# bencebecsy/pta_replicator

Hardware: AMD Instinct MI355X
Metric: realizations/sec, 68 psr x 5000 TOAs GWB+RN+WN (higher is better)
Workload: dtype f64; 1 GPU; BASELINE.json config 3: the 68 pulsars of ng15_dict.json x 5000 synthetic TOAs - HD GWB (gw_log10_A of the dict) + per-pulsar power-law RN (dict values, 30 components) + per-backend EFAC / t2EQUAD / ECORR (dict values), on-chip Philox draws, 1024 realisations per step per GPU; n_toa_total=340000, Nf=3000, npts=600, parallelism=replica-shard x1

## Files before the change

include/pta_replicator_amd.h:

```cpp
#ifndef PTA_REPLICATOR_AMD_H
#define PTA_REPLICATOR_AMD_H

#include <stdint.h>

#ifdef __cplusplus
extern "C" {
#endif

#define PTA_ABI_VERSION 8

#define PTA_OK 0
#define PTA_E_ARG (-1)
#define PTA_E_HIP (-2)
#define PTA_E_NOTPD (-3)

int pta_abi_version(void);
const char *pta_last_error(void);
int pta_device_info(int *cu_count, int *wavefront, char *arch, int arch_len);



int pta_rng_philox_raw(const uint32_t *ctr, const uint32_t *key, int n, uint32_t *out, void *stream);

int pta_rng_fill_normal(uint64_t seed, uint64_t r0, int R, uint32_t stream_id, int npairs, int interleave,
// ... 49 lines not shown
int pta_potrf_batched_ex(double *A, int n, int64_t lda, int64_t strideA, int B, int32_t *info, int flags, void *stream);

int64_t pta_potrf_workspace_doubles(int n, int B, int flags);
int pta_potrf_batched_ws(double *A, int n, int64_t lda, int64_t strideA, int B, int32_t *info, int flags, double *work,
                         int64_t work_doubles, void *stream);

int pta_potrf_warmup(int nchain);

int64_t pta_potrf_ragged_plan_words(int B);
int pta_potrf_ragged_plan(const int32_t *n, const int64_t *off, const int64_t *ld, int B, int flags, int64_t *plan_host,
                          int64_t *work_doubles);
int pta_potrf_ragged(double *A, const int64_t *plan_host, const int64_t *plan_dev, int32_t *info, double *work,
                     int64_t work_doubles, void *stream);



int pta_gwb_twiddle(const double *sqrtC, int Nf, int npts, int i0, double inv_dt, double *T, int64_t ldt, void *stream);

int pta_gwb_idft(const double *w, int64_t ldw, int M, int Nf, const double *T, int64_t ldt, int npts, double *G0,
                 int64_t ldg, int algo, void *stream);

int64_t pta_gwb_twiddle_sym_size(int Nf, int npts, int variant, int64_t *rot_doubles);
int pta_gwb_twiddle_sym(const double *sqrtC, int Nf, int npts, int i0, double inv_dt, double *Tsym, double *rot,
                        int variant, void *stream);
int pta_gwb_idft_rng(uint64_t seed, uint64_t r0, int R, int P, int Nf, const double *Tsym, const double *rot, int npts,
                     double *G0, int64_t ldg, int variant, int rng_fast, void *stream);

int pta_gwb_czt_fits(int Nf, int npts, int i0);
int pta_gwb_czt_setup(const double *sqrtC, int Nf, int npts, int i0, double inv_dt, double *pre, double *FB, double *tw,
                      double *post, void *stream);
int pta_gwb_czt(uint64_t seed, uint64_t r0, const double *w, int64_t ldw, int R, int P, int Nf, int npts, int i0,
                const double *pre, const double *FB, const double *tw, const double *post, double *G0, int64_t ldg,
                int variant, int rng_fast, void *stream);

int pta_gwb_czt_scaled(uint64_t seed, uint64_t r0, const double *w, int64_t ldw, int R, int P, int Nf, int npts, int i0,
                       const double *pre, const double *FB, const double *tw, const double *post, double *G0, int64_t ldg,
                       int variant, int rng_fast, const double *scale, int64_t ld_scale, void *stream);
int pta_gwb_idft_rng_scaled(uint64_t seed, uint64_t r0, int R, int P, int Nf, const double *Tsym, const double *rot, int npts,
                            double *G0, int64_t ldg, int variant, int rng_fast, const double *scale, int64_t ld_scale, void *stream);
int pta_gwb_spectrum_scale(const double *f, const double *hcf0, int Nf, int R, const double *log10_A, const double *gamma, int turnover,
                           double f0, double beta, double power, double *scale, int64_t ld_scale, void *stream);
int pta_gwb_spectrum_scale_user(const int32_t *seg, const double *dx, const double *dxp, const double *hcf0, int Nf, int M, int R,
                                const double *log10_hc, int64_t ld_hc, double *scale, int64_t ld_scale, void *stream);

int pta_gwb_mix(const double *Mchol, int P, const double *G0, int R, int npts, int64_t ldg, double *G, int variant, void *stream);

int pta_gwb_orf_factor(const double *basis, int n_lm, int P, const double *clm, int64_t ld_clm, int R, double *Mchol, int32_t *info,
                       void *stream);
int pta_gwb_mix_batched(const double *Mchol, int64_t ld_m, int P, const double *G0, int R, int npts, int64_t ldg, double *G, int variant,
                        void *stream);

int pta_gwb_bracket(const double *ut, int npts, const double *toa_s, int N, int32_t *jlo, void *stream);

int pta_gwb_weights(const double *ut, int npts, const double *toa_s, const int32_t *jlo, int N, double *w, void *stream);

int pta_gwb_interp(const double *G, int64_t ldg, int P, int npts, const double *ut, const double *toa_s,
                   const int32_t *psr_of_toa, const int32_t *jlo, int N, int R, double scale, double *out,
                   int64_t ld_out, int accumulate, void *stream);

#define PTA_CGW_NPAR 18
int pta_cgw(const double *mjd, int N, const double *par_host, double *out, int accumulate, void *stream);

#define PTA_CW_NPAR 16
int pta_cw_catalog_workspace(int N, int ncw, int64_t *partial_doubles, int *nchunk);
int pta_cw_catalog(const double *mjd, int N, const double *par, int ncw, int psr_term, int mode, double tref,
                   double *partial_ws, double *out, int accumulate, void *stream);
// ... 298 lines not shown
```

pta_replicator_amd/_lib.py:

```python
import ctypes
import os
from ctypes import POINTER, c_char_p, c_double, c_int, c_int32, c_int64, c_uint32, c_uint64, c_void_p

import torch

_HERE = os.path.dirname(os.path.abspath(__file__))
LIB_PATH = os.environ.get("PTA_REPLICATOR_AMD_LIB") or os.path.join(_HERE, "libpta_replicator_amd.so")


class PtaError(RuntimeError):
    """A call into libpta_replicator_amd.so returned a PTA_E_* code."""


if not os.path.exists(LIB_PATH):
    raise ImportError(
        f"{LIB_PATH} is missing: build the HIP library first (python -m pta_replicator_amd.build, or "
        "__graft_entry__.build()). pta_replicator_amd has no CPU fallback.")

lib = ctypes.CDLL(LIB_PATH)

_P = c_void_p


class EnginePlan(ctypes.Structure):
# ... 71 lines not shown
    "pta_rng_fill_normal": (c_int, [c_uint64, c_uint64, c_int, c_uint32, c_int, c_int, _P, _P, c_int64, c_int, _P]),
    "pta_rng_fill_normal_blocks": (c_int, [c_uint64, c_uint64, c_int, c_uint32, c_int, _P, _P, c_int, _P, c_int64, c_int, _P]),
    "pta_rn_basis": (c_int, [_P, c_int, c_double, _P, _P, c_int, c_int, _P, c_int64, _P]),
    "pta_rn_synth": (c_int, [_P, c_int64, c_int, c_int, _P, c_int64, c_int, _P, c_int64, c_int, _P]),
    "pta_wn": (c_int, [_P, _P, _P, c_int, c_int, _P, _P, c_int64, c_int, _P, c_int64, c_int, _P]),
    "pta_quantize_epochs": (c_int, [_P, c_int, c_double, _P, _P, _P, POINTER(c_int)]),
    "pta_dot3_host": (c_int, [_P, c_int64, _P, _P]),
    "pta_pow_host": (c_int, [_P, c_double, c_int64, _P]),
    "pta_legacy_randn": (c_int, [_P, _P, _P, c_int, _P, _P, _P, _P, c_int]),
    "pta_ecorr": (c_int, [_P, _P, c_int, c_int, _P, c_int64, c_int, _P, c_int64, c_int, _P]),
    "pta_orf_pair_arguments": (c_int, [_P, c_int, _P, _P]),
    "pta_orf_hd": (c_int, [_P, c_int, _P, _P]),
    "pta_orf_basis": (c_int, [_P, _P, c_int, c_int, _P, _P]),
    "pta_orf_combine": (c_int, [_P, _P, c_int, c_int, _P, _P]),
    "pta_potrf_batched": (c_int, [_P, c_int, c_int, _P, _P]),
    "pta_potrf_batched_ex": (c_int, [_P, c_int, c_int64, c_int64, c_int, _P, c_int, _P]),
    "pta_potrf_workspace_doubles": (c_int64, [c_int, c_int, c_int]),
    "pta_potrf_batched_ws": (c_int, [_P, c_int, c_int64, c_int64, c_int, _P, c_int, _P, c_int64, _P]),
    "pta_potrf_warmup": (c_int, [c_int]),
    "pta_td_assemble_potrf": (c_int, [_P, _P, c_int, _P, _P, _P, _P, c_int, c_int64, c_int64, c_int, _P, c_int, _P, c_int64, _P]),
    "pta_potrf_ragged_plan_words": (c_int64, [c_int]),
    "pta_potrf_ragged_plan": (c_int, [_P, _P, _P, c_int, c_int, _P, POINTER(c_int64)]),
    "pta_potrf_ragged": (c_int, [_P, _P, _P, _P, _P, c_int64, _P]),
    "pta_gwb_twiddle": (c_int, [_P, c_int, c_int, c_int, c_double, _P, c_int64, _P]),
    "pta_gwb_idft": (c_int, [_P, c_int64, c_int, c_int, _P, c_int64, c_int, _P, c_int64, c_int, _P]),
    "pta_gwb_twiddle_sym_size": (c_int64, [c_int, c_int, c_int, POINTER(c_int64)]),
    "pta_gwb_twiddle_sym": (c_int, [_P, c_int, c_int, c_int, c_double, _P, _P, c_int, _P]),
    "pta_gwb_idft_rng": (c_int, [c_uint64, c_uint64, c_int, c_int, c_int, _P, _P, c_int, _P, c_int64, c_int, c_int, _P]),
    "pta_gwb_czt_fits": (c_int, [c_int, c_int, c_int]),
    "pta_gwb_czt_setup": (c_int, [_P, c_int, c_int, c_int, c_double, _P, _P, _P, _P, _P]),
    "pta_gwb_czt": (c_int, [c_uint64, c_uint64, _P, c_int64, c_int, c_int, c_int, c_int, c_int, _P, _P, _P, _P, _P, c_int64, c_int, c_int, _P]),
    "pta_gwb_czt_scaled": (c_int, [c_uint64, c_uint64, _P, c_int64, c_int, c_int, c_int, c_int, c_int, _P, _P, _P, _P, _P, c_int64, c_int, c_int,
                                   _P, c_int64, _P]),
    "pta_gwb_idft_rng_scaled": (c_int, [c_uint64, c_uint64, c_int, c_int, c_int, _P, _P, c_int, _P, c_int64, c_int, c_int, _P, c_int64, _P]),
    "pta_gwb_spectrum_scale": (c_int, [_P, _P, c_int, c_int, _P, _P, c_int, c_double, c_double, c_double, _P, c_int64, _P]),
    "pta_gwb_mix": (c_int, [_P, c_int, _P, c_int, c_int, c_int64, _P, c_int, _P]),
    "pta_gwb_orf_factor": (c_int, [_P, c_int, c_int, _P, c_int64, c_int, _P, _P, _P]),
    "pta_gwb_mix_batched": (c_int, [_P, c_int64, c_int, _P, c_int, c_int, c_int64, _P, c_int, _P]),
    "pta_gwb_bracket": (c_int, [_P, c_int, _P, c_int, _P, _P]),
    "pta_gwb_weights": (c_int, [_P, c_int, _P, _P, c_int, _P, _P]),
    "pta_gwb_interp": (c_int, [_P, c_int64, c_int, c_int, _P, _P, _P, _P, c_int, c_int, c_double, _P, c_int64, c_int, _P]),
    "pta_cgw": (c_int, [_P, c_int, _P, _P, c_int, _P]),
    "pta_cw_catalog_workspace": (c_int, [c_int, c_int, POINTER(c_int64), POINTER(c_int)]),
    "pta_cw_catalog": (c_int, [_P, c_int, _P, c_int, c_int, c_int, c_double, _P, _P, c_int, _P]),
    "pta_engine_rn_coef": (c_int, [c_uint64, c_uint64, c_int, c_int, c_int, _P, _P, c_int, _P]),
    "pta_engine_generate": (c_int, [POINTER(EnginePlan), POINTER(EngineTables), c_uint64, c_uint64, c_int, _P, c_int64, _P]),
    "pta_hyper_uniform": (c_int, [c_uint64, c_uint64, c_int, c_int, _P, _P, _P, _P]),
    "pta_engine_rn_coef_hyper": (c_int, [c_uint64, c_uint64, c_int, c_int, c_int, _P, _P, _P, _P, _P, _P, c_int, _P]),
    "pta_engine_generate_hyper": (c_int, [POINTER(EnginePlan), POINTER(EngineTables), POINTER(EngineHyper), c_uint64, c_uint64, c_int, _P,
                                          c_int64, _P]),
    "pta_cw_uniform": (c_int, [c_uint64, c_uint64, c_int, c_int, _P, _P, _P, _P]),
    "pta_engine_cw_params": (c_int, [POINTER(CwEngine), c_int, _P]),
    "pta_engine_cw_add": (c_int, [POINTER(EnginePlan), POINTER(CwEngine), c_int, _P, c_int64, c_int, _P]),
    "pta_cw_catalog_uniform": (c_int, [c_uint64, c_uint64, c_int, c_int, _P, _P, _P, _P]),
    "pta_engine_cw_catalog_params": (c_int, [POINTER(CwCatalogEngine), c_int, _P]),
    "pta_engine_cw_catalog_add": (c_int, [POINTER(EnginePlan), POINTER(CwCatalogEngine), c_int, _P, c_int64, c_int, _P]),
    "pta_bwm_uniform": (c_int, [c_uint64, c_uint64, c_int, _P, _P, _P, _P]),
    "pta_engine_bwm_params": (c_int, [POINTER(BwmEngine), c_int, _P]),
    "pta_engine_bwm_add": (c_int, [POINTER(EnginePlan), POINTER(BwmEngine), c_int, _P, c_int64, c_int, _P]),
    "pta_engine_wn_params": (c_int, [POINTER(WnHyper), c_int, _P]),
    "pta_engine_wn_add": (c_int, [POINTER(EnginePlan), POINTER(WnHyper), c_uint64, c_uint64, c_int, _P, c_int64, c_int, _P]),
    "pta_engine_synth": (c_int, [POINTER(EnginePlan), c_uint64, c_uint64, c_int, _P, c_int64, _P]),
    "pta_td_cov_assemble": (c_int, [_P, c_int64, c_int, c_int, _P, _P, _P, _P, _P, c_int64, _P]),
    "pta_td_cov_assemble_all": (c_int, [_P, c_int64, c_int, _P, _P, _P, _P, _P, _P, _P, _P, _P, c_int, c_int, _P]),
    "pta_td_cov_walk_items": (c_int64, [_P, c_int, c_int, c_int, _P]),
    "pta_td_cov_assemble_walk": (c_int, [_P, c_int64, c_int, _P, _P, _P, _P, _P, _P, _P, _P, _P, c_int, _P, c_int64, _P, c_int, _P]),
# ... 79 lines not shown
```

pta_replicator_amd/csrc/pta_czt_kernels.hip:

```cpp
#include "pta_common.h"
#include "pta_fft.h"

__global__ __launch_bounds__(PTA_FFT_THREADS) void k_czt_setup(const double *__restrict__ sqrtC, int Nf, int npts, int i0,
                                                               double inv_dt, double *__restrict__ pre,
                                                               double *__restrict__ FB, double *__restrict__ tw,
                                                               double *__restrict__ post) {
  __shared__ double re[PTA_FFT_PLANE], im[PTA_FFT_PLANE];
  const int tid = threadIdx.x;
  const int Kf = Nf - 2;
  const int64_t n = 2 * (int64_t)Nf - 2;
  for (int m = tid; m < PTA_FFT_N; m += PTA_FFT_THREADS) {
    double s, c;
    sincospi((double)(2 * m) / (double)PTA_FFT_N, &s, &c);
    tw[2 * m] = c;
    tw[2 * m + 1] = -s;
    double pr = 0.0, pi_ = 0.0;
    if (m < Kf) {
      int64_t k = m + 1, q = (k * k) % (2 * n);
      sincospi((double)q / (double)n, &s, &c);
      pr = sqrtC[k] * c;
      pi_ = sqrtC[k] * s;
    }
    pre[2 * m] = pr;
    pre[2 * m + 1] = pi_;
// ... 300 lines not shown
extern "C" int pta_gwb_czt_scaled(uint64_t seed, uint64_t r0, const double *w, int64_t ldw, int R, int P, int Nf, int npts, int i0,
                                  const double *pre, const double *FB, const double *tw, const double *post, double *G0, int64_t ldg,
                                  int variant, int rng_fast, const double *scale, int64_t ld_scale, void *stream) {
  PTA_REQUIRE(pre && FB && tw && post && G0 && scale, PTA_E_ARG, "pta_gwb_czt_scaled: NULL argument");
  PTA_REQUIRE(!w, PTA_E_ARG, "pta_gwb_czt_scaled: draws are generated on chip (w must be NULL)");
  (void)ldw;
  PTA_REQUIRE(R > 0 && P > 0 && P < (1 << 24) && npts > 0 && ldg >= npts, PTA_E_ARG, "pta_gwb_czt_scaled: R=%d P=%d npts=%d", R, P,
              npts);
  PTA_REQUIRE(czt_fits(Nf, npts, i0), PTA_E_ARG, "pta_gwb_czt_scaled: Nf=%d npts=%d i0=%d does not fit one 4096-point convolution", Nf,
              npts, i0);
  PTA_REQUIRE(ld_scale >= Nf - 1, PTA_E_ARG, "pta_gwb_czt_scaled: ld_scale=%lld < Nf - 1", (long long)ld_scale);
  int64_t M64 = (int64_t)R * P;
  PTA_REQUIRE(M64 < (1LL << 31), PTA_E_ARG, "pta_gwb_czt_scaled: R*P too large");
  const int M = (int)M64;
  PTA_REQUIRE(variant == 0 || variant == 1, PTA_E_ARG, "pta_gwb_czt_scaled: variant %d (0 or 1)", variant);
#define PTA_CZT_S(FASTV, FUSEV)                                                                                                     \
  hipLaunchKernelGGL((k_gwb_czt<true, FASTV, FUSEV, true>), dim3(M), dim3(PTA_FFT_THREADS), 0, pta_stream(stream), seed, r0, nullptr, \
                     0, M, P, Nf, npts, i0, pre, FB, tw, post, G0, ldg, scale, ld_scale, czt_last2(npts, i0))
  if (variant == 0) {
    if (rng_fast)
      PTA_CZT_S(true, PTA_CZT_FUSE_DEFAULT);
    else
      PTA_CZT_S(false, PTA_CZT_FUSE_DEFAULT);
  } else {
    if (rng_fast)
      PTA_CZT_S(true, 0);
    else
      PTA_CZT_S(false, 0);
  }
#undef PTA_CZT_S
  PTA_LAUNCH_CHECK();
  return PTA_OK;
}
```

pta_replicator_amd/csrc/pta_engine_kernels.hip:

```cpp
#include "pta_common.h"
#include "pta_rng.h"
#include "pta_mfma.h"

__global__ void k_engine_rn_coef(uint64_t seed, uint64_t r0, int R, int P, int K, const double *__restrict__ amp,
                                 double *__restrict__ coef, int fast) {
  pta_rng_stage_tables();
  __syncthreads();
  int idx = blockIdx.x * blockDim.x + threadIdx.x;
  int hp = K / 2;
  int total = R * P * hp;
  if (idx >= total) return;
  int p = idx % hp, ra = idx / hp;
  int a = ra % P, r = ra / P;
  double z0, z1;
  pta_normal_pair(seed, r0 + (uint64_t)r, pta_stream_id(PTA_STREAM_RN, (uint32_t)a), (uint32_t)p, z0, z1, fast);
  int64_t o = (int64_t)ra * K + 2 * p;
  coef[o] = amp[(int64_t)a * K + 2 * p] * z0;
  coef[o + 1] = amp[(int64_t)a * K + 2 * p + 1] * z1;
}

extern "C" int pta_engine_rn_coef(uint64_t seed, uint64_t r0, int R, int P, int K, const double *amp, double *coef, int rng_fast,
                                  void *stream) {
  PTA_REQUIRE(amp && coef, PTA_E_ARG, "pta_engine_rn_coef: NULL argument");
  PTA_REQUIRE(R > 0 && P > 0 && K > 0 && (K % 2) == 0, PTA_E_ARG, "pta_engine_rn_coef: R=%d P=%d K=%d (K must be even)", R, P, K);
// ... 361 lines not shown
  PTA_REQUIRE(!p.wn_a || p.wn_b, PTA_E_ARG, "pta_engine_synth: wn_b missing");
  PTA_REQUIRE(!p.wn_c || !p.wn_a, PTA_E_ARG, "pta_engine_synth: wn_c (single-deviate white noise) replaces wn_a / wn_b - pass one or the other");
  PTA_REQUIRE(!p.ecorr_toa || p.epoch_of, PTA_E_ARG, "pta_engine_synth: epoch_of missing");
  const int variant = p.synth_variant;
  const bool copies = variant == 16 || variant == 32 || variant == 48 || variant == 64;
  PTA_REQUIRE(variant == 0 || variant == 1 || variant == 2 || variant == 6 || copies || (variant >= 100 && variant <= 164), PTA_E_ARG,
              "pta_engine_synth: synth_variant %d does not exist (0, 1, 2, 6, 16, 32, 48, 64, 100 .. 164)", variant);
  if (variant != 6) {
    const int xcd = variant == 1 ? 0 : 1;
    const unsigned pad = variant >= 100 ? (unsigned)(variant - 100) * 1024u : 0u;
    const int64_t total = (int64_t)pta_cdiv(R, ENG_MR) * p.n_tiles, nwg = ((total + 7) >> 3) << 3;
    PTA_REQUIRE(nwg < (1LL << 31), PTA_E_ARG, "pta_engine_synth: %lld workgroups exceed one launch", (long long)nwg);
    const bool noidx = variant == 2 || (copies && ((variant - 16) & 16));
    const bool rnidx = !noidx && p.rn_k > 0 && p.ldf < (1LL << 28) && ((int64_t)p.rn_k * p.ldf + PTA_ENGINE_TILE) * 8 + 24 < (1LL << 32) &&
                       (int64_t)R * p.n_psr * p.rn_k * 8 < (1LL << 32);
    const bool generic = variant == 2 || (copies && ((variant - 16) & 32));
    const bool all = !generic && p.gw_npts > 0 && (p.wn_a || p.wn_c) && p.ecorr_toa;
    hipLaunchKernelGGL(synth_kernel(p.rng_fast != 0, p.wn_c != nullptr, rnidx, all), dim3((unsigned)nwg), dim3(PTA_ENGINE_TILE), pad,
                       pta_stream(stream), p, seed, r0, R, out, ld_out, xcd);
    PTA_LAUNCH_CHECK();
    return PTA_OK;
  }
  PTA_REQUIRE(!p.wn_c, PTA_E_ARG, "pta_engine_synth: the single-deviate white noise exists in the MFMA kernel only");
  PTA_REQUIRE(p.n_tiles <= 65535, PTA_E_ARG, "pta_engine_synth: %d tiles exceed the 2-D launch of the all-VALU kernel", p.n_tiles);
  hipLaunchKernelGGL(k_engine_synth<6>, dim3(pta_cdiv(R, ENG_RB), p.n_tiles), dim3(PTA_ENGINE_TILE), 0, pta_stream(stream), p, seed, r0, R,
                     out, ld_out, p.rng_fast ? 1 : 0);
  PTA_LAUNCH_CHECK();
  return PTA_OK;
}

extern "C" int pta_gwb_czt(uint64_t seed, uint64_t r0, const double *w, int64_t ldw, int R, int P, int Nf, int npts, int i0,
                           const double *pre, const double *FB, const double *tw, const double *post, double *G0, int64_t ldg,
                           int variant, int rng_fast, void *stream);
extern "C" int pta_gwb_idft_rng(uint64_t seed, uint64_t r0, int R, int P, int Nf, const double *Tsym, const double *rot, int npts,
                                double *G0, int64_t ldg, int variant, int rng_fast, void *stream);
extern "C" int pta_gwb_mix(const double *Mchol, int P, const double *G0, int R, int npts, int64_t ldg, double *G, int variant,
                           void *stream);
extern "C" int pta_gwb_mix_batched(const double *Mchol, int64_t ld_m, int P, const double *G0, int R, int npts, int64_t ldg, double *G,
                                   int variant, void *stream);

static int engine_generate(const char *fn, const pta_engine_plan *plan_host, const pta_engine_tables *tables_host,
                           const pta_engine_hyper *hyper, uint64_t seed, uint64_t r0, int R, double *out, int64_t ld_out, void *stream) {
  PTA_REQUIRE(plan_host && tables_host && out, PTA_E_ARG, "%s: NULL argument", fn);
  const pta_engine_hyper fixed{};
  const pta_engine_hyper &h = hyper ? *hyper : fixed;
  pta_engine_plan p = *plan_host;
  const pta_engine_tables &tb = *tables_host;
  int rc;
  if (p.rn_k > 0) {
    PTA_REQUIRE(tb.rn_amp && tb.ws_coef, PTA_E_ARG, "%s: red-noise amplitudes / workspace missing", fn);
    if (h.rn_log10_A) {
      PTA_REQUIRE(h.rn_gamma && h.rn_f && h.rn_tspan, PTA_E_ARG, "%s: rn_gamma / rn_f / rn_tspan missing", fn);
      rc = pta_engine_rn_coef_hyper(seed, r0, R, p.n_psr, p.rn_k, h.rn_f, h.rn_tspan, h.rn_log10_A, h.rn_gamma, tb.rn_amp, tb.ws_coef,
                                    p.rng_fast, stream);
    } else {
      rc = pta_engine_rn_coef(seed, r0, R, p.n_psr, p.rn_k, tb.rn_amp, tb.ws_coef, p.rng_fast, stream);
    }
    if (rc != PTA_OK) return rc;
    p.rn_coef = tb.ws_coef;
  }
  if (p.gw_npts > 0) {
    PTA_REQUIRE(tb.Mchol && tb.ws_G0 && tb.ws_G, PTA_E_ARG, "%s: GWB factor / workspace missing", fn);
    const double *scale = h.gw_scale;
    if (!scale && h.gw_log10_A) {
      PTA_REQUIRE(h.gw_gamma && h.gw_f && h.gw_hcf0 && h.ws_scale, PTA_E_ARG, "%s: gw_gamma / gw_f / gw_hcf0 / ws_scale missing", fn);
      rc = pta_gwb_spectrum_scale(h.gw_f, h.gw_hcf0, tb.gw_nf, R, h.gw_log10_A, h.gw_gamma, h.gw_turnover, h.gw_f0, h.gw_beta,
                                  h.gw_power, h.ws_scale, h.ld_gw_scale, stream);
      if (rc != PTA_OK) return rc;
      scale = h.ws_scale;
    }
    if (tb.use_czt) {
      PTA_REQUIRE(tb.czt_pre && tb.czt_FB && tb.czt_tw && tb.czt_post, PTA_E_ARG, "%s: chirp-z tables missing", fn);
      rc = scale ? pta_gwb_czt_scaled(seed, r0, nullptr, 0, R, p.n_psr, tb.gw_nf, p.gw_npts, tb.gw_i0, tb.czt_pre, tb.czt_FB, tb.czt_tw,
                                      tb.czt_post, tb.ws_G0, p.gw_npts, tb.czt_variant, p.rng_fast, scale, h.ld_gw_scale, stream)
                 : pta_gwb_czt(seed, r0, nullptr, 0, R, p.n_psr, tb.gw_nf, p.gw_npts, tb.gw_i0, tb.czt_pre, tb.czt_FB, tb.czt_tw,
                               tb.czt_post, tb.ws_G0, p.gw_npts, tb.czt_variant, p.rng_fast, stream);
    } else {
      PTA_REQUIRE(tb.Tsym && tb.rot, PTA_E_ARG, "%s: DFT-GEMM tables missing", fn);
      rc = scale ? pta_gwb_idft_rng_scaled(seed, r0, R, p.n_psr, tb.gw_nf, tb.Tsym, tb.rot, p.gw_npts, tb.ws_G0, p.gw_npts, tb.idft_variant,
                                           p.rng_fast, scale, h.ld_gw_scale, stream)
                 : pta_gwb_idft_rng(seed, r0, R, p.n_psr, tb.gw_nf, tb.Tsym, tb.rot, p.gw_npts, tb.ws_G0, p.gw_npts, tb.idft_variant,
                                    p.rng_fast, stream);
    }
    if (rc != PTA_OK) return rc;
    rc = h.gw_mchol ? pta_gwb_mix_batched(h.gw_mchol, h.ld_gw_mchol, p.n_psr, tb.ws_G0, R, p.gw_npts, p.gw_npts, tb.ws_G, tb.mix_variant, stream)
                    : pta_gwb_mix(tb.Mchol, p.n_psr, tb.ws_G0, R, p.gw_npts, p.gw_npts, tb.ws_G, tb.mix_variant, stream);
    if (rc != PTA_OK) return rc;
    p.gw_G = tb.ws_G;
  }
  return pta_engine_synth(&p, seed, r0, R, out, ld_out, stream);
}

extern "C" int pta_engine_generate(const pta_engine_plan *plan_host, const pta_engine_tables *tables_host, uint64_t seed, uint64_t r0,
                                   int R, double *out, int64_t ld_out, void *stream) {
  return engine_generate("pta_engine_generate", plan_host, tables_host, nullptr, seed, r0, R, out, ld_out, stream);
}

extern "C" int pta_engine_generate_hyper(const pta_engine_plan *plan_host, const pta_engine_tables *tables_host,
                                         const pta_engine_hyper *hyper_host, uint64_t seed, uint64_t r0, int R, double *out,
                                         int64_t ld_out, void *stream) {
  PTA_REQUIRE(hyper_host, PTA_E_ARG, "pta_engine_generate_hyper: NULL argument");
  return engine_generate("pta_engine_generate_hyper", plan_host, tables_host, hyper_host, seed, r0, R, out, ld_out, stream);
}
```

pta_replicator_amd/csrc/pta_fft.h:

```cpp
#pragma once
#include "pta_rng.h"

#define PTA_FFT_N 4096
#define PTA_FFT_THREADS 512
#define PTA_FFT_PHYS(i) ((i) + ((i) >> 3) + (((i) >> 9) << 3))
#define PTA_FFT_PLANE (PTA_FFT_N + PTA_FFT_N / 8 + 64)

struct pta_cplx {
  double re, im;
};

PTA_HD pta_cplx pta_cmul(pta_cplx a, pta_cplx b) { return {fma(a.re, b.re, -(a.im * b.im)), fma(a.re, b.im, a.im * b.re)}; }
PTA_HD pta_cplx pta_cadd(pta_cplx a, pta_cplx b) { return {a.re + b.re, a.im + b.im}; }
PTA_HD pta_cplx pta_csub(pta_cplx a, pta_cplx b) { return {a.re - b.re, a.im - b.im}; }
template <bool INV>
PTA_HD pta_cplx pta_cmuli(pta_cplx a) {
  return INV ? pta_cplx{-a.im, a.re} : pta_cplx{a.im, -a.re};
}

template <bool INV>
PTA_HD void pta_dft8(pta_cplx *v) {
  const double h = 0.70710678118654752440;
  pta_cplx a0 = pta_cadd(v[0], v[4]), a4 = pta_csub(v[0], v[4]);
  pta_cplx a1 = pta_cadd(v[1], v[5]), a5 = pta_csub(v[1], v[5]);
// ... 115 lines not shown
  pta_cplx d0 = pta_cadd(a4, t6), d1 = pta_cadd(t5, t7);
  v[1] = pta_cadd(d0, d1);
}

template <int LOG2S>
PTA_HD void pta_fft_core_inv_out01(pta_cplx *v, const pta_cplx *w) {
  if (LOG2S > 0) {
#pragma unroll
    for (int q = 1; q < 8; ++q) v[q] = pta_cmul(v[q], pta_cplx{w[q].re, -w[q].im});
  }
  pta_dft8_inv_out01(v);
}

template <bool INV, int LOG2S>
PTA_HD void pta_fft_pass_w(double *re, double *im, int tid, const pta_cplx *w) {
  int b, o;
  pta_fft_map<LOG2S>(tid, b, o);
  pta_cplx v[8];
  pta_fft_load<LOG2S>(re, im, b, o, v);
  pta_fft_core<INV, LOG2S>(v, w);
  pta_fft_store<LOG2S>(re, im, b, o, v);
}

template <bool INV, int LOG2S, int TW = 3>
PTA_HD void pta_fft_pass(double *re, double *im, const double *tw, int tid) {
  int b, o;
  pta_fft_map<LOG2S>(tid, b, o);
  pta_cplx v[8], w[8];
  pta_fft_twiddles<LOG2S, TW>(tw, o, w);
  pta_fft_load<LOG2S>(re, im, b, o, v);
  pta_fft_core<INV, LOG2S>(v, w);
  pta_fft_store<LOG2S>(re, im, b, o, v);
}
```

pta_replicator_amd/engine.py:

```python
import ctypes

import numpy as np
import torch

from . import _bwm, _cw, _hyper, _lib, _wn_hyper, device as dv
from . import deterministic as det
from . import red_noise as rn
from . import spharmORFbasis as anis
from . import white_noise as wn
from ._position import ra_dec
from .constants import DAY_IN_SEC, YEAR_IN_SEC
from .engine_bwm import BwmStatisticMixin
from .engine_fstat import FStatisticMixin
from .engine_lnl import LikelihoodMixin
from .engine_os import OptimalStatisticMixin
from .engine_td import TimeDomainMixin
from .engine_terms import PerRealisationTermsMixin

STREAM_GWB, STREAM_RN, STREAM_WN, STREAM_ECORR, STREAM_TD, STREAM_TDGW = 1, 2, 3, 4, 5, 6
STREAM_HYPER = 7
STREAM_CW = 8
STREAM_BWM = 9


# ... 204 lines not shown
        pl.n_tiles = len(t_psr)
        pl.tile_psr, pl.tile_start, pl.tile_count, pl.tile_ep0, pl.tile_epn = [x.data_ptr() for x in self.d_tiles]

        pl.gw_npts = 0
        if self._gw is not None:
            c = self._gw
            grid = rn.gwb_time_grid(self.psrs_ideal_view(), c["npts"], c["howml"])
            self.grid = grid
            npts, Nf = grid["npts"], grid["Nf"]
            ORF = rn.gwb_orf_device(self.psrs, c["no_correlations"], c["clm"], c["lmax"])
            self.ORF = ORF.clone()
            self.d_M = rn.cholesky_device(ORF)
            self.d_orf_basis = None
            if _hyper.n_lm(c) is not None:
                self.d_orf_basis = anis.correlated_basis_device(rn.pulsar_locations(self.psrs), int(c["lmax"]))
            self.C = rn.gwb_spectrum(grid["f"], grid["dur"], c["howml"], c["A"], c["g"], c["turnover"], c["f0"], c["beta"],
                                     c["power"], c["userSpec"])
            self.ldt = rn.pad16(npts)
            self.d_T = dv.empty((2 * (Nf - 2), self.ldt))
            sqrtC = dv.f64(self.C ** 0.5)
            _lib.call("pta_gwb_twiddle", dv.ptr(sqrtC), Nf, npts, 10, ctypes.c_double(1.0 / grid["dt"]), dv.ptr(self.d_T), self.ldt, s)
            nrot = ctypes.c_int64(0)
            nsym = _lib.lib.pta_gwb_twiddle_sym_size(Nf, npts, self.idft_variant, ctypes.byref(nrot))
            self._idft_variant_built = self.idft_variant
            self.d_Tsym, self.d_rot = dv.empty((nsym,)), dv.empty((nrot.value,))
            _lib.call("pta_gwb_twiddle_sym", dv.ptr(sqrtC), Nf, npts, 10, ctypes.c_double(1.0 / grid["dt"]), dv.ptr(self.d_Tsym),
                      dv.ptr(self.d_rot), self.idft_variant, s)
            self.use_czt = bool(_lib.lib.pta_gwb_czt_fits(Nf, npts, 10)) and self.gwb_transform != "gemm"
            self.d_czt = None
            if self.use_czt:
                self.d_czt = [dv.empty((2 * 4096,)), dv.empty((2 * 4096,)), dv.empty((2 * 4096,)), dv.empty((2 * npts,))]
                _lib.call("pta_gwb_czt_setup", dv.ptr(sqrtC), Nf, npts, 10, ctypes.c_double(1.0 / grid["dt"]),
                          *[dv.ptr(x) for x in self.d_czt], s)
            self.d_ut = dv.f64(grid["ut"])
            self.d_jlo = dv.empty((N,), dtype=torch.int32)
            _lib.call("pta_gwb_bracket", dv.ptr(self.d_ut), npts, dv.ptr(self.d_toa_s), N, dv.ptr(self.d_jlo), s)
            torch.cuda.current_stream().synchronize()
            self.d_gw_w = dv.empty((N,))
            _lib.call("pta_gwb_weights", dv.ptr(self.d_ut), npts, dv.ptr(self.d_toa_s), dv.ptr(self.d_jlo), N, dv.ptr(self.d_gw_w), s)
            torch.cuda.current_stream().synchronize()
            pl.gw_npts, pl.gw_jlo, pl.gw_w = npts, self.d_jlo.data_ptr(), self.d_gw_w.data_ptr()

        pl.det = None
        extra = getattr(self, "_delays", None)
        if self._det or extra is not None:
            self.d_det = dv.zeros((N,)) if extra is None else dv.f64(extra)
            mjd_all = dv.f64(np.concatenate(self.mjd)) if self._det else None
            for kw in self._det or []:
                for a in range(P):
                    ra, dec = ra_dec(self.psrs[a])
                    par, _, _, _ = det.cgw_parameters(np.pi / 2 - dec, ra, **{k: v for k, v in kw.items() if k != "signal_name"})
                    par = np.ascontiguousarray(par)
                    o = int(self.off[a])
                    _lib.call("pta_cgw", ctypes.c_void_p(mjd_all.data_ptr() + 8 * o), len(self.mjd[a]), dv.hptr(par),
                              ctypes.c_void_p(self.d_det.data_ptr() + 8 * o), 1, s)
            if self._det:
                torch.cuda.current_stream().synchronize()
            pl.det = self.d_det.data_ptr()
        self._prepared = True
        if self._wn is not None and getattr(self, "td_warmup", True):
            _lib.call("pta_potrf_warmup", 2)
        return self

    def psrs_ideal_view(self):
        class _V:
            pass
# ... 5 lines not shown
            v.toas.last_MJD = _V()
            v.toas.first_MJD.value = float(m.min())
            v.toas.last_MJD.value = float(m.max())
            out.append(v)
        return out

    def _pick(self, val, a):
        if val is None or np.isscalar(val):
            return val
        if len(val) != self.P:
            raise ValueError(f"expected a scalar or one entry per pulsar ({self.P}), got {len(val)}")
        return val[a]

    def _pick_flags(self, flags, a):
        if flags is None:
            return None
        if len(flags) != self.P:
            raise ValueError("flags must be a per-pulsar list of flag lists")
        return flags[a]

    def workspace(self, R):
        ws = getattr(self, "_ws", None)
        if ws is None or ws["R"] < R:
            ws = {"R": R}
            tb = _lib.EngineTables()
            if self.plan.rn_k:
                ws["coef"] = dv.empty((R, self.P, self.K))
                tb.rn_amp, tb.ws_coef = self.d_amp.data_ptr(), ws["coef"].data_ptr()
            if self.plan.gw_npts:
                ws["G0"] = dv.empty((R, self.P, self.plan.gw_npts))
                ws["G"] = dv.empty((R, self.P, self.plan.gw_npts))
                tb.Mchol, tb.ws_G0, tb.ws_G = self.d_M.data_ptr(), ws["G0"].data_ptr(), ws["G"].data_ptr()
                tb.gw_nf, tb.gw_i0 = self.grid["Nf"], 10
                if getattr(self, "d_czt", None) is not None:
                    tb.czt_pre, tb.czt_FB, tb.czt_tw, tb.czt_post = (x.data_ptr() for x in self.d_czt)
                tb.Tsym, tb.rot = self.d_Tsym.data_ptr(), self.d_rot.data_ptr()
                tb.idft_variant = self._idft_variant_built
            ws["tables"] = tb
            self._ws = ws
        ws["tables"].czt_variant, ws["tables"].mix_variant = int(self.czt_variant), int(self.mix_variant)
        if self.plan.gw_npts:
            if self.use_czt and getattr(self, "d_czt", None) is None:
                raise ValueError("use_czt was switched on after prepare(): the chirp-z tables were not built")
            ws["tables"].use_czt = 1 if self.use_czt else 0
        self.plan.rng_fast, self.plan.synth_variant = int(self.rng_fast), int(self.synth_variant)
        return ws

    def max_batch(self, hyper=False, cw=False, clm=False):
        per_real = 8 * self.P * ((self.K if self.plan.rn_k else 0) + 2 * self.plan.gw_npts)
        if hyper and self.plan.gw_npts:
            per_real += 8 * self.grid["Nf"]
        cap = 65536
        if clm:
            per_real += 8 * self.P * self.P + 4
            cap = 65535
        if cw:
            S = 1 if cw is True else int(cw)
            if S < 1:
                raise ValueError(f"max_batch: cw must be True, False or a source count >= 1, got {cw!r}")
            per_real += 8 * (self.P * S * _lib.CW_ENGINE_NPAR + _cw.N_SRC * S + self.P)
            cap = min(cap, ((1 << 31) - 1) // (self.P * S))
        return int(max(1 if cap < 16 else 16, min(cap, self.workspace_bytes // max(per_real, 1))))

    def generate(self, R, r0=0, out=None, theta=None):
        hyper, cw = self._theta_parts(theta, R)
        return self._generate(R, r0, out, hyper, cw)

    def _generate(self, R, r0, out, hyper, cw, mask_unconfigured=True, raise_orf=True):
        if not self._prepared:
            self.prepare()
        dev = None if hyper is None else self._theta_device(hyper, R, mask_unconfigured)
        if out is None:
            out = dv.empty((R, self.n_toa))
        clm = None if dev is None else dev[_hyper.CLM_KEY]
# ... 483 lines not shown
```

Baseline: 217,100 realizations/s.

## Add half-length chirp-z GWB kernel packing real spectrum into two 2048-point convolutions

Adds a chirp-z variant that exploits the Hermitian symmetry of the real GWB signal. It packs the spectrum into one half-size complex sequence, so the convolution runs as two 2048-point halves instead of a full 4096-point transform. Output samples are written in even/odd pairs from a single inverse half transform. The setup kernel builds the matching pre/post/twiddle tables. The engine routes to it when czt_variant is 2 and the sizes fit, which adds table memory and a new code path to maintain.

```diff
diff --git a/include/pta_replicator_amd.h b/include/pta_replicator_amd.h
--- a/include/pta_replicator_amd.h
+++ b/include/pta_replicator_amd.h
@@ -105,6 +105,16 @@
 int pta_gwb_czt(uint64_t seed, uint64_t r0, const double *w, int64_t ldw, int R, int P, int Nf, int npts, int i0,
                 const double *pre, const double *FB, const double *tw, const double *post, double *G0, int64_t ldg,
                 int variant, int rng_fast, void *stream);
+
+int pta_gwb_czt_half_fits(int Nf, int npts, int i0);
+int pta_gwb_czt_half_setup(const double *sqrtC, int Nf, int npts, int i0, double inv_dt, double *pre, double *FB, double *tw,
+                           double *post, void *stream);
+int pta_gwb_czt_half(uint64_t seed, uint64_t r0, const double *w, int64_t ldw, int R, int P, int Nf, int npts, int i0,
+                     const double *pre, const double *FB, const double *tw, const double *post, double *G0, int64_t ldg,
+                     int variant, int rng_fast, void *stream);
+int pta_gwb_czt_half_scaled(uint64_t seed, uint64_t r0, const double *w, int64_t ldw, int R, int P, int Nf, int npts, int i0,
+                            const double *pre, const double *FB, const double *tw, const double *post, double *G0, int64_t ldg,
+                            int variant, int rng_fast, const double *scale, int64_t ld_scale, void *stream);
 
 int pta_gwb_czt_scaled(uint64_t seed, uint64_t r0, const double *w, int64_t ldw, int R, int P, int Nf, int npts, int i0,
                        const double *pre, const double *FB, const double *tw, const double *post, double *G0, int64_t ldg,
diff --git a/pta_replicator_amd/_lib.py b/pta_replicator_amd/_lib.py
--- a/pta_replicator_amd/_lib.py
+++ b/pta_replicator_amd/_lib.py
@@ -127,6 +127,12 @@
     "pta_gwb_czt": (c_int, [c_uint64, c_uint64, _P, c_int64, c_int, c_int, c_int, c_int, c_int, _P, _P, _P, _P, _P, c_int64, c_int, c_int, _P]),
     "pta_gwb_czt_scaled": (c_int, [c_uint64, c_uint64, _P, c_int64, c_int, c_int, c_int, c_int, c_int, _P, _P, _P, _P, _P, c_int64, c_int, c_int,
                                    _P, c_int64, _P]),
+    "pta_gwb_czt_half_fits": (c_int, [c_int, c_int, c_int]),
+    "pta_gwb_czt_half_setup": (c_int, [_P, c_int, c_int, c_int, c_double, _P, _P, _P, _P, _P]),
+    "pta_gwb_czt_half": (c_int, [c_uint64, c_uint64, _P, c_int64, c_int, c_int, c_int, c_int, c_int, _P, _P, _P, _P, _P, c_int64, c_int, c_int,
+                                 _P]),
+    "pta_gwb_czt_half_scaled": (c_int, [c_uint64, c_uint64, _P, c_int64, c_int, c_int, c_int, c_int, c_int, _P, _P, _P, _P, _P, c_int64, c_int,
+                                        c_int, _P, c_int64, _P]),
     "pta_gwb_idft_rng_scaled": (c_int, [c_uint64, c_uint64, c_int, c_int, c_int, _P, _P, c_int, _P, c_int64, c_int, c_int, _P, c_int64, _P]),
     "pta_gwb_spectrum_scale": (c_int, [_P, _P, c_int, c_int, _P, _P, c_int, c_double, c_double, c_double, _P, c_int64, _P]),
     "pta_gwb_mix": (c_int, [_P, c_int, _P, c_int, c_int, c_int64, _P, c_int, _P]),
diff --git a/pta_replicator_amd/csrc/pta_czt_kernels.hip b/pta_replicator_amd/csrc/pta_czt_kernels.hip
--- a/pta_replicator_amd/csrc/pta_czt_kernels.hip
+++ b/pta_replicator_amd/csrc/pta_czt_kernels.hip
@@ -356,3 +356,291 @@
   PTA_LAUNCH_CHECK();
   return PTA_OK;
 }
+
+static bool czt_half_fits(int Nf, int npts, int i0) {
+  if (!czt_fits(Nf, npts, i0)) return false;
+  const int64_t Kf = (int64_t)Nf - 2, nm = ((int64_t)npts + 2) / 2;
+  return (Kf + 1) / 2 + nm - 1 <= PTA_FFT_N2;
+}
+
+extern "C" int pta_gwb_czt_half_fits(int Nf, int npts, int i0) { return czt_half_fits(Nf, npts, i0) ? 1 : 0; }
+
+struct czt_half_geom {
+  int Kf, K0, K1, m0, par, nm;
+};
+static __host__ __device__ czt_half_geom czt_half_geometry(int Nf, int npts, int i0) {
+  czt_half_geom g;
+  g.Kf = Nf - 2;
+  g.K0 = (g.Kf + 1) / 2;
+  g.K1 = g.Kf - g.K0;
+  g.m0 = i0 >> 1;
+  g.par = i0 & 1;
+  g.nm = (i0 + npts - 1) / 2 - g.m0 + 1;
+  return g;
+}
+
+__global__ __launch_bounds__(PTA_FFT_THREADS) void k_czt_half_setup(const double *__restrict__ sqrtC, int Nf, int npts, int i0,
+                                                                    double inv_dt, double *__restrict__ pre, double *__restrict__ FB,
+                                                                    double *__restrict__ tw, double *__restrict__ post) {
+  __shared__ double re[PTA_FFT_PLANE], im[PTA_FFT_PLANE];
+  const int tid = threadIdx.x;
+  const czt_half_geom g = czt_half_geometry(Nf, npts, i0);
+  const int64_t n2 = (int64_t)Nf - 1;
+  for (int m = tid; m < PTA_FFT_N; m += PTA_FFT_THREADS) {
+    double s, c;
+    if (m < PTA_FFT_N2) {
+      sincospi((double)(2 * m) / (double)PTA_FFT_N, &s, &c);
+      tw[2 * m] = c;
+      tw[2 * m + 1] = -s;
+      double orr = 0.0, oi = 0.0;
+      if (m < g.K0) {
+        sincospi((double)(m + 1) / (double)n2, &s, &c);
+        orr = -s;
+        oi = c;
+      }
+      tw[2 * (PTA_FFT_N2 + m)] = orr;
+      tw[2 * (PTA_FFT_N2 + m) + 1] = oi;
+    }
+    double pr = 0.0, pi_ = 0.0;
+    if (m < g.Kf) {
+      int64_t k = m + 1, q = (k * k) % (2 * n2);
+      sincospi((double)q / (double)n2, &s, &c);
+      pr = 0.5 * sqrtC[k] * c;
+      pi_ = 0.5 * sqrtC[k] * s;
+    }
+    pre[2 * m] = pr;
+    pre[2 * m + 1] = pi_;
+    const int h = m >> 11, p = m & (PTA_FFT_N2 - 1);
+    const int Kb = h ? g.K1 : g.K0, kb = h ? g.K0 : 0;
+    int64_t d = p;
+    bool used = Kb > 0 && p < g.nm;
+    if (!used && Kb > 0 && p >= PTA_FFT_N2 - (Kb - 1)) {
+      d = (int64_t)p - PTA_FFT_N2;
+      used = true;
+    }
+    double br = 0.0, bi = 0.0;
+    if (used) {
+      int64_t e = (int64_t)g.m0 - kb - 1 + d, q = (e * e) % (2 * n2);
+      sincospi((double)q / (double)n2, &s, &c);
+      br = c;
+      bi = -s;
+    }
+    re[PTA_FFT_PHYS(m)] = br;
+    im[PTA_FFT_PHYS(m)] = bi;
+  }
+  for (int ss = tid; ss < g.nm; ss += PTA_FFT_THREADS) {
+    int64_t m = (int64_t)g.m0 + ss, q = (m * m) % (2 * n2);
+    double s, c;
+    sincospi((double)q / (double)n2, &s, &c);
+    double amp = 2.0 * inv_dt / (double)(2 * n2);
+    post[2 * ss] = amp * c;
+    post[2 * ss + 1] = amp * s;
+  }
+  __threadfence_block();
+  __syncthreads();
+  {
+    pta_cplx w4[4];
+    pta_fft4_twiddles(tw, tid, w4);
+    for (int h = 0; h < 2; ++h) {
+      pta_cplx v[4];
+      pta_fft4_load(re, im, h, tid, v);
+      pta_fft4_core<false>(v, w4);
+      pta_fft4_store(re, im, h, tid, v);
+    }
+  }
+  __syncthreads();
+  pta_fft_pass<false, 6>(re, im, tw, tid);
+  __syncthreads();
+  pta_fft_pass<false, 3>(re, im, tw, tid);
+  __syncthreads();
+  pta_fft_pass<false, 0>(re, im, tw, tid);
+  __syncthreads();
+  for (int m = tid; m < PTA_FFT_N; m += PTA_FFT_THREADS) {
+    const int slot = (m & 7) * (PTA_FFT_N / 8) + (m >> 3);
+    FB[2 * slot] = re[PTA_FFT_PHYS(m)] * (1.0 / PTA_FFT_N2);
+    FB[2 * slot + 1] = im[PTA_FFT_PHYS(m)] * (1.0 / PTA_FFT_N2);
+  }
+}
+
+extern "C" int pta_gwb_czt_half_setup(const double *sqrtC, int Nf, int npts, int i0, double inv_dt, double *pre, double *FB, double *tw,
+                                      double *post, void *stream) {
+  PTA_REQUIRE(sqrtC && pre && FB && tw && post, PTA_E_ARG, "pta_gwb_czt_half_setup: NULL argument");
+  PTA_REQUIRE(czt_half_fits(Nf, npts, i0), PTA_E_ARG, "pta_gwb_czt_half_setup: Nf=%d npts=%d i0=%d does not fit two 2048-point convolutions",
+              Nf, npts, i0);
+  hipLaunchKernelGGL(k_czt_half_setup, dim3(1), dim3(PTA_FFT_THREADS), 0, pta_stream(stream), sqrtC, Nf, npts, i0, inv_dt, pre, FB, tw,
+                     post);
+  PTA_LAUNCH_CHECK();
+  return PTA_OK;
+}
+
+template <bool RNG, bool FAST, bool SCALED>
+__global__ __launch_bounds__(PTA_FFT_THREADS, 4) void k_gwb_czt_half(uint64_t seed, uint64_t r0, const double *__restrict__ w, int64_t ldw,
+                                                                       int P, int Nf, int npts, int i0, const double *__restrict__ pre,
+                                                                       const double *__restrict__ FB, const double *__restrict__ tw,
+                                                                       const double *__restrict__ post, double *__restrict__ G0,
+                                                                       int64_t ldg, const double *__restrict__ scale, int64_t ld_scale) {
+  __shared__ double re[PTA_FFT_PLANE], im[PTA_FFT_PLANE];
+  const int tid = threadIdx.x;
+  const int row = blockIdx.x;
+  const czt_half_geom g = czt_half_geometry(Nf, npts, i0);
+  if (RNG) {
+    pta_rng_stage_tables();
+    __syncthreads();
+  }
+  const uint64_t real = r0 + (uint64_t)(row / P);
+  const uint32_t strm = pta_stream_id(PTA_STREAM_GWB, (uint32_t)(row % P));
+  const pta_cplx *pre2 = reinterpret_cast<const pta_cplx *>(pre);
+  const pta_cplx *om2 = reinterpret_cast<const pta_cplx *>(tw) + PTA_FFT_N2;
+  const double sg = ((Nf - 1) & 1) ? -1.0 : 1.0;
+  const double *twi = tw;
+  asm volatile("" : "+s"(twi));
+  auto draw = [&](int k, double &wr, double &wi) {
+    if (RNG) {
+      pta_normal_pair(seed, real, strm, (uint32_t)k, wr, wi, FAST ? 1 : 0);
+    } else {
+      wr = w[(int64_t)row * ldw + 2 * k];
+      wi = w[(int64_t)row * ldw + 2 * k + 1];
+    }
+    if (SCALED) {
+      const double sc = scale[(int64_t)(row / P) * ld_scale + k];
+      wr *= sc;
+      wi *= sc;
+    }
+  };
+  pta_cplx v[4];
+#pragma unroll
+  for (int q = 0; q < 4; ++q) {
+    const int t = tid + 512 * q;
+    v[q] = {0.0, 0.0};
+    if (t < g.K0) {
+      const int k = t + 1, km = g.Kf - t;
+      pta_cplx x, xm;
+      draw(k, x.re, x.im);
+      xm = x;
+      if (t < g.K1) draw(km, xm.re, xm.im);
+      const pta_cplx pk = pre2[k - 1], pm = pre2[km - 1], om = om2[t];
+      const pta_cplx A = pta_cmul(pk, x), B = pta_cmul(pta_cplx{sg * pm.re, sg * pm.im}, pta_cplx{xm.re, -xm.im});
+      v[q] = pta_cadd(pta_cadd(A, B), pta_cmul(om, pta_csub(A, B)));
+      if (t < g.K1) {
+        const pta_cplx Am = pta_cmul(pm, xm), Bm = pta_cmul(pta_cplx{sg * pk.re, sg * pk.im}, pta_cplx{x.re, -x.im});
+        const pta_cplx am = pta_cadd(pta_cadd(Am, Bm), pta_cmul(pta_cplx{om.re, -om.im}, pta_csub(Am, Bm)));
+        const int pm1 = PTA_FFT_PHYS(PTA_FFT_N2 + g.K1 - 1 - t);
+        re[pm1] = am.re;
+        im[pm1] = am.im;
+      }
+    }
+    if (t >= g.K1) {
+      const int pz = PTA_FFT_PHYS(PTA_FFT_N2 + t);
+      re[pz] = 0.0;
+      im[pz] = 0.0;
+    }
+  }
+  __syncthreads();
+  {
+    pta_cplx w4[4], v1[4];
+    pta_fft4_twiddles(tw, tid, w4);
+    pta_fft4_core<false>(v, w4);
+    pta_fft4_store(re, im, 0, tid, v);
+    pta_fft4_load(re, im, 1, tid, v1);
+    pta_fft4_core<false>(v1, w4);
+    pta_fft4_store(re, im, 1, tid, v1);
+  }
+  __syncthreads();
+  pta_fft_pass<false, 6, 1>(re, im, tw, tid);
+  __syncthreads();
+  pta_fft_pass<false, 3, 1>(re, im, tw, tid);
+  __syncthreads();
+  if (tid < 256) {
+    pta_cplx y[8], y1[8];
+    const pta_cplx *fb = reinterpret_cast<const pta_cplx *>(FB) + tid;
+    pta_fft_load<0>(re, im, tid, 0, y);
+    pta_dft8<false>(y);
+#pragma unroll
+    for (int q = 0; q < 8; ++q) y[q] = pta_cmul(y[q], fb[q * (PTA_FFT_N / 8)]);
+    pta_fft_load<0>(re, im, 256 + tid, 0, y1);
+    pta_dft8<false>(y1);
+#pragma unroll
+    for (int q = 0; q < 8; ++q) y[q] = pta_cadd(y[q], pta_cmul(y1[q], fb[q * (PTA_FFT_N / 8) + 256]));
+    pta_dft8<true>(y);
+    pta_fft_store<0>(re, im, tid, 0, y);
+  }
+  __syncthreads();
+  if (tid < 256) pta_fft_pass<true, 3, 1>(re, im, twi, tid);
+  __syncthreads();
+  if (tid < 256) pta_fft_pass_at<true, 6, 1>(re, im, twi, tid >> 6, tid & 63);
+  __syncthreads();
+  const pta_cplx *post2 = reinterpret_cast<const pta_cplx *>(post);
+  auto put = [&](int s, pta_cplx z) {
+    const pta_cplx pp = post2[s];
+    const pta_cplx x = pta_cmul(z, pp);
+    const int jj = 2 * s - g.par;
+    if (jj >= 0 && jj < npts) G0[(int64_t)row * ldg + jj] = x.re;
+    if (jj + 1 < npts) G0[(int64_t)row * ldg + jj + 1] = x.im;
+  };
+  if (g.nm <= 512) {
+    if (tid < g.nm) {
+      pta_cplx w4[4], y[4];
+      pta_fft4_twiddles(twi, tid, w4);
+      pta_fft4_load(re, im, 0, tid, y);
+      pta_fft4_core_inv_out0(y, w4);
+      put(tid, y[0]);
+    }
+  } else {
+    pta_cplx w4[4], y[4];
+    pta_fft4_twiddles(twi, tid, w4);
+    pta_fft4_load(re, im, 0, tid, y);
+    pta_fft4_core<true>(y, w4);
+#pragma unroll
+    for (int q = 0; q < 4; ++q)
+      if (tid + 512 * q < g.nm) put(tid + 512 * q, y[q]);
+  }
+}
+
+static int czt_half_launch(const char *fn, uint64_t seed, uint64_t r0, const double *w, int64_t ldw, int R, int P, int Nf, int npts, int i0,
+                           const double *pre, const double *FB, const double *tw, const double *post, double *G0, int64_t ldg, int variant,
+                           int rng_fast, const double *scale, int64_t ld_scale, void *stream) {
+  PTA_REQUIRE(pre && FB && tw && post && G0, PTA_E_ARG, "%s: NULL argument", fn);
+  PTA_REQUIRE(R > 0 && P > 0 && P < (1 << 24) && npts > 0 && ldg >= npts, PTA_E_ARG, "%s: R=%d P=%d npts=%d", fn, R, P, npts);
+  PTA_REQUIRE(czt_half_fits(Nf, npts, i0), PTA_E_ARG, "%s: Nf=%d npts=%d i0=%d does not fit two 2048-point convolutions", fn, Nf, npts, i0);
+  PTA_REQUIRE(variant == 0, PTA_E_ARG, "%s: variant %d (0: the kernel has one form)", fn, variant);
+  int64_t M64 = (int64_t)R * P;
+  PTA_REQUIRE(M64 < (1LL << 31), PTA_E_ARG, "%s: R*P too large", fn);
+  const int M = (int)M64;
+#define PTA_CZT_H(RNGV, FASTV, SCALEDV)                                                                                                   \
+  hipLaunchKernelGGL((k_gwb_czt_half<RNGV, FASTV, SCALEDV>), dim3(M), dim3(PTA_FFT_THREADS), 0, pta_stream(stream), seed, r0, w, ldw, P, \
+                     Nf, npts, i0, pre, FB, tw, post, G0, ldg, scale, ld_scale)
+  if (scale) {
+    if (rng_fast)
+      PTA_CZT_H(true, true, true);
+    else
+      PTA_CZT_H(true, false, true);
+  } else if (w) {
+    PTA_CZT_H(false, false, false);
+  } else if (rng_fast) {
+    PTA_CZT_H(true, true, false);
+  } else {
+    PTA_CZT_H(true, false, false);
+  }
+#undef PTA_CZT_H
+  PTA_LAUNCH_CHECK();
+  return PTA_OK;
+}
+
+extern "C" int pta_gwb_czt_half(uint64_t seed, uint64_t r0, const double *w, int64_t ldw, int R, int P, int Nf, int npts, int i0,
+                                const double *pre, const double *FB, const double *tw, const double *post, double *G0, int64_t ldg,
+                                int variant, int rng_fast, void *stream) {
+  PTA_REQUIRE(!w || ldw == 0 || ldw >= 2 * (int64_t)Nf, PTA_E_ARG, "pta_gwb_czt_half: ldw too small");
+  return czt_half_launch("pta_gwb_czt_half", seed, r0, w, ldw, R, P, Nf, npts, i0, pre, FB, tw, post, G0, ldg, variant, rng_fast, nullptr, 0,
+                         stream);
+}
+
+extern "C" int pta_gwb_czt_half_scaled(uint64_t seed, uint64_t r0, const double *w, int64_t ldw, int R, int P, int Nf, int npts, int i0,
+                                       const double *pre, const double *FB, const double *tw, const double *post, double *G0, int64_t ldg,
+                                       int variant, int rng_fast, const double *scale, int64_t ld_scale, void *stream) {
+  PTA_REQUIRE(scale, PTA_E_ARG, "pta_gwb_czt_half_scaled: NULL argument");
+  PTA_REQUIRE(!w, PTA_E_ARG, "pta_gwb_czt_half_scaled: draws are generated on chip (w must be NULL)");
+  (void)ldw;
+  PTA_REQUIRE(ld_scale >= Nf - 1, PTA_E_ARG, "pta_gwb_czt_half_scaled: ld_scale=%lld < Nf - 1", (long long)ld_scale);
+  return czt_half_launch("pta_gwb_czt_half_scaled", seed, r0, nullptr, 0, R, P, Nf, npts, i0, pre, FB, tw, post, G0, ldg, variant, rng_fast,
+                         scale, ld_scale, stream);
+}
diff --git a/pta_replicator_amd/csrc/pta_engine_kernels.hip b/pta_replicator_amd/csrc/pta_engine_kernels.hip
--- a/pta_replicator_amd/csrc/pta_engine_kernels.hip
+++ b/pta_replicator_amd/csrc/pta_engine_kernels.hip
@@ -417,6 +417,12 @@
 extern "C" int pta_gwb_czt(uint64_t seed, uint64_t r0, const double *w, int64_t ldw, int R, int P, int Nf, int npts, int i0,
                            const double *pre, const double *FB, const double *tw, const double *post, double *G0, int64_t ldg,
                            int variant, int rng_fast, void *stream);
+extern "C" int pta_gwb_czt_half(uint64_t seed, uint64_t r0, const double *w, int64_t ldw, int R, int P, int Nf, int npts, int i0,
+                                const double *pre, const double *FB, const double *tw, const double *post, double *G0, int64_t ldg,
+                                int variant, int rng_fast, void *stream);
+extern "C" int pta_gwb_czt_half_scaled(uint64_t seed, uint64_t r0, const double *w, int64_t ldw, int R, int P, int Nf, int npts, int i0,
+                                       const double *pre, const double *FB, const double *tw, const double *post, double *G0, int64_t ldg,
+                                       int variant, int rng_fast, const double *scale, int64_t ld_scale, void *stream);
 extern "C" int pta_gwb_idft_rng(uint64_t seed, uint64_t r0, int R, int P, int Nf, const double *Tsym, const double *rot, int npts,
                                 double *G0, int64_t ldg, int variant, int rng_fast, void *stream);
 extern "C" int pta_gwb_mix(const double *Mchol, int P, const double *G0, int R, int npts, int64_t ldg, double *G, int variant,
@@ -456,10 +462,16 @@
     }
     if (tb.use_czt) {
       PTA_REQUIRE(tb.czt_pre && tb.czt_FB && tb.czt_tw && tb.czt_post, PTA_E_ARG, "%s: chirp-z tables missing", fn);
-      rc = scale ? pta_gwb_czt_scaled(seed, r0, nullptr, 0, R, p.n_psr, tb.gw_nf, p.gw_npts, tb.gw_i0, tb.czt_pre, tb.czt_FB, tb.czt_tw,
-                                      tb.czt_post, tb.ws_G0, p.gw_npts, tb.czt_variant, p.rng_fast, scale, h.ld_gw_scale, stream)
-                 : pta_gwb_czt(seed, r0, nullptr, 0, R, p.n_psr, tb.gw_nf, p.gw_npts, tb.gw_i0, tb.czt_pre, tb.czt_FB, tb.czt_tw,
-                               tb.czt_post, tb.ws_G0, p.gw_npts, tb.czt_variant, p.rng_fast, stream);
+      if (tb.czt_variant == 2)
+        rc = scale ? pta_gwb_czt_half_scaled(seed, r0, nullptr, 0, R, p.n_psr, tb.gw_nf, p.gw_npts, tb.gw_i0, tb.czt_pre, tb.czt_FB,
+                                             tb.czt_tw, tb.czt_post, tb.ws_G0, p.gw_npts, 0, p.rng_fast, scale, h.ld_gw_scale, stream)
+                   : pta_gwb_czt_half(seed, r0, nullptr, 0, R, p.n_psr, tb.gw_nf, p.gw_npts, tb.gw_i0, tb.czt_pre, tb.czt_FB, tb.czt_tw,
+                                      tb.czt_post, tb.ws_G0, p.gw_npts, 0, p.rng_fast, stream);
+      else
+        rc = scale ? pta_gwb_czt_scaled(seed, r0, nullptr, 0, R, p.n_psr, tb.gw_nf, p.gw_npts, tb.gw_i0, tb.czt_pre, tb.czt_FB, tb.czt_tw,
+                                        tb.czt_post, tb.ws_G0, p.gw_npts, tb.czt_variant, p.rng_fast, scale, h.ld_gw_scale, stream)
+                   : pta_gwb_czt(seed, r0, nullptr, 0, R, p.n_psr, tb.gw_nf, p.gw_npts, tb.gw_i0, tb.czt_pre, tb.czt_FB, tb.czt_tw,
+                                 tb.czt_post, tb.ws_G0, p.gw_npts, tb.czt_variant, p.rng_fast, stream);
     } else {
       PTA_REQUIRE(tb.Tsym && tb.rot, PTA_E_ARG, "%s: DFT-GEMM tables missing", fn);
       rc = scale ? pta_gwb_idft_rng_scaled(seed, r0, R, p.n_psr, tb.gw_nf, tb.Tsym, tb.rot, p.gw_npts, tb.ws_G0, p.gw_npts, tb.idft_variant,
diff --git a/pta_replicator_amd/csrc/pta_fft.h b/pta_replicator_amd/csrc/pta_fft.h
--- a/pta_replicator_amd/csrc/pta_fft.h
+++ b/pta_replicator_amd/csrc/pta_fft.h
@@ -171,3 +171,63 @@
   pta_fft_core<INV, LOG2S>(v, w);
   pta_fft_store<LOG2S>(re, im, b, o, v);
 }
+
+template <bool INV, int LOG2S, int TW = 3>
+PTA_HD void pta_fft_pass_at(double *re, double *im, const double *tw, int b, int o) {
+  pta_cplx v[8], w[8];
+  pta_fft_twiddles<LOG2S, TW>(tw, o, w);
+  pta_fft_load<LOG2S>(re, im, b, o, v);
+  pta_fft_core<INV, LOG2S>(v, w);
+  pta_fft_store<LOG2S>(re, im, b, o, v);
+}
+
+#define PTA_FFT_N2 2048
+
+template <bool INV>
+PTA_HD void pta_dft4(pta_cplx *v) {
+  pta_cplx c0 = pta_cadd(v[0], v[2]), c2 = pta_csub(v[0], v[2]), c1 = pta_cadd(v[1], v[3]), c3 = pta_cmuli<INV>(pta_csub(v[1], v[3]));
+  v[0] = pta_cadd(c0, c1);
+  v[2] = pta_csub(c0, c1);
+  v[1] = pta_cadd(c2, c3);
+  v[3] = pta_csub(c2, c3);
+}
+
+PTA_HD void pta_fft4_twiddles(const double *tw, int o, pta_cplx *w) {
+  w[1] = reinterpret_cast<const pta_cplx *>(tw)[2 * o];
+  w[2] = pta_cmul(w[1], w[1]);
+  w[3] = pta_cmul(w[1], w[2]);
+}
+
+PTA_HD void pta_fft4_load(const double *re, const double *im, int h, int o, pta_cplx *v) {
+  const int p0 = PTA_FFT_PHYS(PTA_FFT_N2 * h + o);
+#pragma unroll
+  for (int q = 0; q < 4; ++q) v[q] = {re[p0 + q * pta_fft_stride<9>::QSTEP], im[p0 + q * pta_fft_stride<9>::QSTEP]};
+}
+
+PTA_HD void pta_fft4_store(double *re, double *im, int h, int o, const pta_cplx *v) {
+  const int p0 = PTA_FFT_PHYS(PTA_FFT_N2 * h + o);
+#pragma unroll
+  for (int q = 0; q < 4; ++q) {
+    re[p0 + q * pta_fft_stride<9>::QSTEP] = v[q].re;
+    im[p0 + q * pta_fft_stride<9>::QSTEP] = v[q].im;
+  }
+}
+
+template <bool INV>
+PTA_HD void pta_fft4_core(pta_cplx *v, const pta_cplx *w) {
+  if (INV) {
+#pragma unroll
+    for (int q = 1; q < 4; ++q) v[q] = pta_cmul(v[q], pta_cplx{w[q].re, -w[q].im});
+  }
+  pta_dft4<INV>(v);
+  if (!INV) {
+#pragma unroll
+    for (int q = 1; q < 4; ++q) v[q] = pta_cmul(v[q], w[q]);
+  }
+}
+
+PTA_HD void pta_fft4_core_inv_out0(pta_cplx *v, const pta_cplx *w) {
+#pragma unroll
+  for (int q = 1; q < 4; ++q) v[q] = pta_cmul(v[q], pta_cplx{w[q].re, -w[q].im});
+  v[0] = pta_cadd(pta_cadd(v[0], v[2]), pta_cadd(v[1], v[3]));
+}
diff --git a/pta_replicator_amd/engine.py b/pta_replicator_amd/engine.py
--- a/pta_replicator_amd/engine.py
+++ b/pta_replicator_amd/engine.py
@@ -260,6 +260,11 @@
                 self.d_czt = [dv.empty((2 * 4096,)), dv.empty((2 * 4096,)), dv.empty((2 * 4096,)), dv.empty((2 * npts,))]
                 _lib.call("pta_gwb_czt_setup", dv.ptr(sqrtC), Nf, npts, 10, ctypes.c_double(1.0 / grid["dt"]),
                           *[dv.ptr(x) for x in self.d_czt], s)
+            self.d_czt_half = None
+            if self.use_czt and _lib.lib.pta_gwb_czt_half_fits(Nf, npts, 10):
+                self.d_czt_half = [dv.empty((2 * 4096,)), dv.empty((2 * 4096,)), dv.empty((2 * 4096,)), dv.empty((2 * npts,))]
+                _lib.call("pta_gwb_czt_half_setup", dv.ptr(sqrtC), Nf, npts, 10, ctypes.c_double(1.0 / grid["dt"]),
+                          *[dv.ptr(x) for x in self.d_czt_half], s)
             self.d_ut = dv.f64(grid["ut"])
             self.d_jlo = dv.empty((N,), dtype=torch.int32)
             _lib.call("pta_gwb_bracket", dv.ptr(self.d_ut), npts, dv.ptr(self.d_toa_s), N, dv.ptr(self.d_jlo), s)
@@ -331,14 +336,21 @@
                 ws["G"] = dv.empty((R, self.P, self.plan.gw_npts))
                 tb.Mchol, tb.ws_G0, tb.ws_G = self.d_M.data_ptr(), ws["G0"].data_ptr(), ws["G"].data_ptr()
                 tb.gw_nf, tb.gw_i0 = self.grid["Nf"], 10
-                if getattr(self, "d_czt", None) is not None:
-                    tb.czt_pre, tb.czt_FB, tb.czt_tw, tb.czt_post = (x.data_ptr() for x in self.d_czt)
                 tb.Tsym, tb.rot = self.d_Tsym.data_ptr(), self.d_rot.data_ptr()
                 tb.idft_variant = self._idft_variant_built
             ws["tables"] = tb
             self._ws = ws
-        ws["tables"].czt_variant, ws["tables"].mix_variant = int(self.czt_variant), int(self.mix_variant)
+        variant, czt = int(self.czt_variant), getattr(self, "d_czt", None)
+        if variant == 2:
+            if getattr(self, "d_czt_half", None) is not None:
+                czt = self.d_czt_half
+            else:
+                variant = 0
+        ws["tables"].czt_variant, ws["tables"].mix_variant = variant, int(self.mix_variant)
         if self.plan.gw_npts:
+            if czt is not None:
+                tb = ws["tables"]
+                tb.czt_pre, tb.czt_FB, tb.czt_tw, tb.czt_post = (x.data_ptr() for x in czt)
             if self.use_czt and getattr(self, "d_czt", None) is None:
                 raise ValueError("use_czt was switched on after prepare(): the chirp-z tables were not built")
             ws["tables"].use_czt = 1 if self.use_czt else 0
```

New measurement: 214,400 realizations/s. 1.2% lower.
